# CapAI/ship-sim-gym

Hardware: AMD Instinct MI355X
Metric: env steps/sec (batched ShipEnv) (higher is better)
Workload: dtype f64

## Files before the change

### ship_sim_gym_amd/csrc/shipsim_kernels.hip

```cpp
#include <hip/hip_runtime.h>

#include <cfloat>
#include <cstdint>
#include <type_traits>

#include "shipsim.h"
#include "shipsim_internal.h"

namespace ssg {

__device__ __forceinline__ double *lds_base()
{
    extern __shared__ double s_lds[];
    return s_lds;
}

__device__ __forceinline__ double dmin(double a, double b) { return __builtin_fmin(a, b); }
__device__ __forceinline__ double dmax(double a, double b) { return __builtin_fmax(a, b); }

__device__ __forceinline__ double obs_fma(double a, double b, double c)
{
#ifndef SSG_NO_LIDAR_FMA
    return __builtin_fma(a, b, c);
#else
// ... 93 lines not shown
            const double dx = px - x, dy = py - y;
            const double d = obs_fma(dx, dx, dy * dy);
            const bool take = ((gm >> g) & 1u) & (d < best);
            best = take ? d : best;
            gi = take ? g : gi;
        }
        if (gi >= 0) { gx = hG[(2 * gi) * ld]; gy = hG[(2 * gi + 1) * ld]; }
        return;
    }
    for (int g = 0; g < c.n_goals; ++g) {
        const double px = goal_at<LDS_BANK, DYN>(c, goff, g, 0);
        const double py = goal_at<LDS_BANK, DYN>(c, goff, g, 1);
        const double dx = px - x, dy = py - y;
        const double d = obs_fma(dx, dx, dy * dy);
        const bool take = ((gm >> g) & 1u) & (d < best);
        best = take ? d : best;
        gi = take ? g : gi;
    }
    if (gi >= 0) { gx = goal_at<LDS_BANK, DYN>(c, goff, gi, 0); gy = goal_at<LDS_BANK, DYN>(c, goff, gi, 1); }
}

__device__ __forceinline__ void nearest_goal_regs(int n_goals, unsigned gm, double x, double y, const double *gp, double &gx, double &gy)
{
    gx = -1.0;
    gy = -1.0;
    double best = INFINITY;
#pragma unroll
    for (int g = 0; g < SSG_MAX_GOALS; ++g) {
        const double px = gp[2 * g], py = gp[2 * g + 1];
        const double dx = px - x, dy = py - y;
        const double d = obs_fma(dx, dx, dy * dy);
        const bool take = (g < n_goals) & (bool)((gm >> g) & 1u) & (d < best);
        best = take ? d : best;
        gx = take ? px : gx;
        gy = take ? py : gy;
    }
}

__device__ __forceinline__ int next_map(const DevCfg &c, int map_id, int env)
{
    if (c.map_ring > 0) {
        const int base = env * c.map_ring;
        const int nxt = map_id + 1;
        return (nxt - base >= c.map_ring) ? base : nxt;
    }
    const int nxt = map_id + 1;
    return (nxt >= c.n_maps) ? 0 : nxt;
}

__device__ __forceinline__ void beam_end(double cx, double cy, double ca, double sa, double cphi, double sphi, double dist,
                                         double &ex, double &ey)
{
    const double ux = obs_fma(ca, cphi, -(sa * sphi)), uy = obs_fma(sa, cphi, ca * sphi);
    ex = obs_fma(dist, ux, cx);
    ey = obs_fma(dist, uy, cy);
}

__host__ __device__ __forceinline__ constexpr int nb_lo(int nb) { return (nb + 1) / 2; }
constexpr int kBeamTabBytes = 2 * SSG_MAX_BEAMS * 8;
constexpr int kShipTabBytes = 6 * 8 * 8;
constexpr int kTrafficTabBytes = SSG_N_TRAFFIC * 4 * 8 * 8;
constexpr int kPoseDoubles = 7;
constexpr int kGoalScratchBytes = 64 * SSG_MAX_GOALS * 2 + 64 * 4;
constexpr int kTrafficScratchBytes = 64 * SSG_N_TRAFFIC * 2 + 64 * 4;
__host__ __device__ __forceinline__ constexpr int lds_fixed_bytes(int epw, bool dyn)
{
    return kBeamTabBytes + kShipTabBytes + (dyn ? kTrafficTabBytes : 0) + kPoseDoubles * epw * 8 + (dyn ? 8 : 6) * epw * 4 + 4 * (epw / 64) * 4 +
           (epw / 64) * (kGoalScratchBytes + (dyn ? kTrafficScratchBytes : 0));
}
__host__ __device__ __forceinline__ constexpr int lds_res_bytes(int nb) { return nb * 64 * 8; }
__host__ __device__ __forceinline__ constexpr int lds_queue_bytes(int nb0) { return (2 * nb0 * 64 + 64) * 2; }
__host__ __device__ __forceinline__ constexpr int lds_tile_bytes(int nb)
{
    return 2 * lds_res_bytes(nb) + 2 * lds_queue_bytes(nb_lo(nb));
}

constexpr int kHdrLidar = 10, kHdrGoals = 2 * SSG_MAX_GOALS;
static_assert(SSG_MAP_OFF_COUNTS == 0 && SSG_MAP_OFF_AABB == 2 && SSG_MAP_OFF_GOALS == kHdrLidar && SSG_MAP_OFF_SPAWN_GOAL == kHdrLidar + kHdrGoals,
              "the record's head: counts, boxes, goals, spawn goal");
#ifndef SSG_SIX_ROLE_MAX_EPW
#define SSG_SIX_ROLE_MAX_EPW 128
#endif
__host__ __device__ __forceinline__ constexpr int tile_roles(int epw, bool dyn) { return (epw <= SSG_SIX_ROLE_MAX_EPW && !dyn) ? 6 : 4; }
__host__ __device__ __forceinline__ constexpr int lds_hdr_bytes(int epw, bool lds_bank, bool dyn) { return lds_bank ? 0 : ((tile_roles(epw, dyn) - 2) * kHdrLidar + kHdrGoals) * epw * 8; }

constexpr unsigned long long kLidarMiss = ~0ull;

template <bool LDS_BANK> struct PlaneChunk { static constexpr int n = LDS_BANK ? 4 : 8; };

template <bool EXACT>
__device__ __forceinline__ double seg_mad(double a, double b, double c) { return EXACT ? a * b + c : obs_fma(a, b, c); }

template <bool LDS_BANK, bool EXACT>
__device__ __forceinline__ void lidar_pass(const DevCfg &c, const int n_items, const unsigned short *queue,
                                           unsigned long long *res , const double *beamtab,
                                           const double cx, const double cy, const double ca, const double sa,
                                           const int rec_off, const int lane, const double *hLt = nullptr , const int ld = 0)
{
    for (int base = 0; base < n_items; base += 64) {
        const int idx = base + lane;
        const bool act = idx < n_items;
        const unsigned code = queue[act ? idx : 0];
        const int src = code & 63, bi = (code >> 6) & (SSG_MAX_BEAMS - 1), s = (code >> 10) & 1;
        const double wcx = __shfl(cx, src), wcy = __shfl(cy, src), wca = __shfl(ca, src), wsa = __shfl(sa, src);
        const int woff = __shfl(rec_off, src);
        double ex, ey;
        beam_end(wcx, wcy, wca, wsa, beamtab[bi], beamtab[SSG_MAX_BEAMS + bi], c.lidar_dist, ex, ey);
        int cnt;
        if constexpr (LDS_BANK) cnt = (int)bank_at<LDS_BANK>(c, woff + SSG_MAP_OFF_COUNTS + s);
        else cnt = (int)hLt[s * ld + src];
        const int pb = woff + SSG_MAP_OFF_PLANES + s * (SSG_MAX_HULL * SSG_PLANE_DOUBLES);
        bool outside = false;
        bool out_sure = false, maybe = false;
        constexpr double kSignEps = 1e-9;
        bool ok = false;
        double ptx = ex, pty = ey;
        double bd = -1.0, bden = 1.0, t_hit = 0.0;
        int bj = 0;
        constexpr int kPlaneChunk = PlaneChunk<LDS_BANK>::n;
        for (int j0 = 0; __any(act & (j0 < cnt)); j0 += kPlaneChunk) {
            double pv0x[kPlaneChunk], pv0y[kPlaneChunk], pnx[kPlaneChunk], pny[kPlaneChunk], pv0n[kPlaneChunk];
            double pdtmin[kPlaneChunk], pdtmax[kPlaneChunk];
#pragma unroll
            for (int u = 0; u < kPlaneChunk; ++u) {
                const int j = j0 + u;
                const int q = pb + SSG_PLANE_DOUBLES * ((j < SSG_MAX_HULL) ? j : 0);
                const bool want = LDS_BANK || (act & (j < cnt));
                pv0x[u] = pv0y[u] = pnx[u] = pny[u] = pv0n[u] = 0.0;
                if (EXACT && want) { const double2 vv = bank_at2<LDS_BANK>(c, q + 0); pv0x[u] = vv.x; pv0y[u] = vv.y; }
                if (want) { const double2 nn = bank_at2<LDS_BANK>(c, q + 2); pnx[u] = nn.x; pny[u] = nn.y; }
                if (want) pv0n[u] = bank_at<LDS_BANK>(c, q + 4);
                if (EXACT) {
                    const int jp = (j == 0) ? cnt - 1 : j - 1;
                    const int qp = pb + SSG_PLANE_DOUBLES * ((jp >= 0 && jp < SSG_MAX_HULL) ? jp : 0);
                    const double ux = bank_at<LDS_BANK>(c, qp + 0), uy = bank_at<LDS_BANK>(c, qp + 1);
                    pdtmin[u] = seg_mad<EXACT>(pnx[u], uy, -(pny[u] * ux));
                    pdtmax[u] = seg_mad<EXACT>(pnx[u], pv0y[u], -(pny[u] * pv0x[u]));
                }
            }
#pragma unroll
            for (int u = 0; u < kPlaneChunk; ++u) {
                const int j = j0 + u;
                const bool valid = act & (j < cnt);
                const double nx = pnx[u], ny = pny[u], v0n = pv0n[u];
                const double an = seg_mad<EXACT>(wcx, nx, wcy * ny);
                const double d = an - v0n;
                if (EXACT) {
                    outside = outside | (valid & ((nx * (wcx - pv0x[u]) + ny * (wcy - pv0y[u])) > 0.0));
                } else {
                    out_sure = out_sure | (valid & (d > kSignEps));
                    maybe = maybe | (valid & !(d < -kSignEps));
                }
                const bool front = valid & !(d < 0.0);
                const double bn = seg_mad<EXACT>(ex, nx, ey * ny);
                const double den = dmax(an - bn, DBL_MIN);
                if (EXACT) {
                    const double t = d / den;
                    const double omt = 1.0 - t;
                    const double qx = seg_mad<EXACT>(ex, t, wcx * omt), qy = seg_mad<EXACT>(ey, t, wcy * omt);
                    const double dtv = seg_mad<EXACT>(nx, qy, -(ny * qx));
                    const bool acc = front & !((t < 0.0) | (1.0 < t)) & (pdtmin[u] <= dtv) & (dtv <= pdtmax[u]);
                    ok = ok | acc;
                    ptx = acc ? qx : ptx;
                    pty = acc ? qy : pty;
                } else {
                    const bool better = front & (d <= den) & (d * bden >= bd * den);
// ... 47 lines not shown
        }
#ifdef SSG_LIDAR_COUNT
        if (c.dbg) {
            const unsigned long long ma = __ballot(act), mh = __ballot(hit), mo = __ballot(act & !outside);
            if (lane == 0) { atomicAdd(c.dbg + 65536 + 0, (unsigned long long)__popcll(ma)); atomicAdd(c.dbg + 65536 + 1, (unsigned long long)__popcll(mh));
                             atomicAdd(c.dbg + 65536 + 2, 1ull); atomicAdd(c.dbg + 65536 + 3, (unsigned long long)__popcll(mo)); }
        }
#endif
    }
}

template <class T>
__device__ __forceinline__ void st_out(T *p, T v)
{
#ifdef SSG_WT
    __hip_atomic_store(p, v, __ATOMIC_RELAXED, __HIP_MEMORY_SCOPE_AGENT);
#else
    *p = v;
#endif
}

#ifdef SSG_STAMPS
#define SSG_STAMP(k)                                                                              \
    do {                                                                                          \
        __builtin_amdgcn_sched_barrier(0);                                                        \
        unsigned long long t_;                                                                    \
        asm volatile("s_memtime %0\n\ts_waitcnt lgkmcnt(0)" : "=s"(t_)::"memory");               \
        __builtin_amdgcn_sched_barrier(0);                                                        \
        stamp_[k] = t_;                                                                           \
    } while (0)
#define SSG_STAMP_FLUSH(n)                                                                        \
    do {                                                                                          \
        if (c.dbg && lane == 0) {                                                                 \
            unsigned long long *d_ = c.dbg + 16 * (size_t)(blockIdx.x * (NR * EPW / 64) + (threadIdx.x >> 6)); \
            for (int k_ = 0; k_ < 16; ++k_) d_[k_] = stamp_[k_];   \
        }                                                                                         \
    } while (0)
#ifdef SSG_STAMPS_ITER
#define SSG_STAMP_K(i) do { } while (0)
#else
#define SSG_STAMP_K(i) do { if (k == (K >= 2 ? K - 2 : 0)) SSG_STAMP(i); } while (0)
#endif
#else
#define SSG_STAMP(k) do { } while (0)
#define SSG_STAMP_K(i) do { } while (0)
#define SSG_STAMP_FLUSH(n) do { } while (0)
#endif

#ifdef SSG_STAMPS
#define SSG_CLOCK_BEGIN() do { } while (0)
#define SSG_CLOCK_END() do { } while (0)
#else
#define SSG_CLOCK_BEGIN() const unsigned long long clk_c0_ = __builtin_amdgcn_s_memtime(), clk_r0_ = __builtin_amdgcn_s_memrealtime()
#define SSG_CLOCK_END()                                                                            \
    do {                                                                                           \
        if (c.dbg && blockIdx.x == 0 && threadIdx.x == 0) {                                        \
            c.dbg[0] = __builtin_amdgcn_s_memtime() - clk_c0_;                                     \
            c.dbg[1] = __builtin_amdgcn_s_memrealtime() - clk_r0_;                                 \
        }                                                                                          \
    } while (0)
#endif

#ifdef SSG_ABLATION
#define SSG_ABL(bit) (c.flags & (1u << (16 + (bit))))
#else
#define SSG_ABL(bit) false
#endif

__device__ __forceinline__ void ship_world(const double *shiptab, double ca, double sa, double x, double y,
                                           double (&swx)[SSG_SHIP_VERTS], double (&swy)[SSG_SHIP_VERTS], double &sbl,
                                           double &sbr, double &sbb, double &sbt)
{
    sbl = INFINITY; sbr = -INFINITY; sbb = INFINITY; sbt = -INFINITY;
#pragma unroll
    for (int i = 0; i < SSG_SHIP_VERTS; ++i) {
        const double hx = shiptab[0 * 8 + i], hy = shiptab[1 * 8 + i];
        swx[i] = ca * hx + (-sa) * hy + x;
        swy[i] = sa * hx + ca * hy + y;
        sbl = dmin(sbl, swx[i]); sbr = dmax(sbr, swx[i]);
        sbb = dmin(sbb, swy[i]); sbt = dmax(sbt, swy[i]);
    }
}

template <int NB, bool LDS_BANK, bool EXACT>
__device__ __forceinline__ void lidar_query(const DevCfg &c, unsigned long long *res, unsigned short *queue,
                                            const double *beamtab, const int b_first, const int b_count, const double cx,
                                            const double cy, const double ca, const double sa, const int rec_off,
                                            const bool live, const int lane, const double *hL = nullptr , const int ld = 0)
{
    constexpr int NB0 = nb_lo(NB);
    constexpr int kTrash = 2 * NB0 * 64;
    int n_items = 0;
    const double eps = 1e-6;
    double al[2], ab[2], ar[2], at[2];
#pragma unroll
    for (int s = 0; s < 2; ++s) {
        double2 lb, rt;
        if constexpr (LDS_BANK) {
            lb = bank_at2<LDS_BANK>(c, rec_off + SSG_MAP_OFF_AABB + 4 * s + 0);
            rt = bank_at2<LDS_BANK>(c, rec_off + SSG_MAP_OFF_AABB + 4 * s + 2);
        } else {
            lb.x = hL[(SSG_MAP_OFF_AABB + 4 * s + 0) * ld]; lb.y = hL[(SSG_MAP_OFF_AABB + 4 * s + 1) * ld];
            rt.x = hL[(SSG_MAP_OFF_AABB + 4 * s + 2) * ld]; rt.y = hL[(SSG_MAP_OFF_AABB + 4 * s + 3) * ld];
        }
        al[s] = lb.x - eps;
        ab[s] = lb.y - eps;
        ar[s] = rt.x + eps;
        at[s] = rt.y + eps;
    }
    (void)ab; (void)at; (void)al; (void)ar;
#ifdef SSG_QUEUE_BEAM_MAJOR
#pragma unroll
    for (int k = 0; k < NB0; ++k) {
        if (k < b_count) {
            const int i = b_first + k;
            res[i * 64 + lane] = kLidarMiss;
            if (!SSG_ABL(1)) {
                double ex, ey;
                beam_end(cx, cy, ca, sa, beamtab[i], beamtab[SSG_MAX_BEAMS + i], c.lidar_dist, ex, ey);
                const double lox = dmin(cx, ex), hix = dmax(cx, ex), loy = dmin(cy, ey), hiy = dmax(cy, ey);
#pragma unroll
                for (int s = 0; s < 2; ++s) {
                    const bool need = live & (lox <= ar[s]) & (al[s] <= hix) & (loy <= at[s]) & (ab[s] <= hiy);
                    const unsigned long long m = __ballot(need);
                    const int pos = n_items + (int)__builtin_amdgcn_mbcnt_hi((unsigned)(m >> 32),
                                                                              __builtin_amdgcn_mbcnt_lo((unsigned)m, 0u));
                    queue[need ? pos : (kTrash + lane)] = (unsigned short)(lane | (k << 6) | (s << 10));
                    n_items += __popcll(m);
                }
            }
        }
    }
#else
    unsigned needmask = 0u;
    const double lca = c.lidar_dist * ca, lsa = c.lidar_dist * sa;
    const bool org0 = live & (cx <= ar[0]), org1 = live & (al[1] <= cx);
#pragma unroll
    for (int k = 0; k < NB0; ++k) {
        if (k < b_count) {
            const int i = b_first + k;
            res[i * 64 + lane] = kLidarMiss;
            if (!SSG_ABL(1)) {
                const double ex = obs_fma(lca, beamtab[i], obs_fma(-lsa, beamtab[SSG_MAX_BEAMS + i], cx));
                needmask |= (org0 | (live & (ex <= ar[0]))) ? (1u << (2 * k + 0)) : 0u;
                needmask |= (org1 | (live & (al[1] <= ex))) ? (1u << (2 * k + 1)) : 0u;
            }
        }
    }
    {
        const int cnt = __popc(needmask);
        int incl = cnt;
        incl += __builtin_amdgcn_update_dpp(0, incl, 0x111, 0xF, 0xF, false);
        incl += __builtin_amdgcn_update_dpp(0, incl, 0x112, 0xF, 0xF, false);
        incl += __builtin_amdgcn_update_dpp(0, incl, 0x114, 0xF, 0xF, false);
        incl += __builtin_amdgcn_update_dpp(0, incl, 0x118, 0xF, 0xF, false);
        incl += __builtin_amdgcn_update_dpp(0, incl, 0x142, 0xA, 0xF, false);
        incl += __builtin_amdgcn_update_dpp(0, incl, 0x143, 0xC, 0xF, false);
        n_items = __builtin_amdgcn_readlane(incl, 63);
        int pos = incl - cnt;
#pragma unroll
        for (int k = 0; k < NB0; ++k) {
            if (k < b_count) {
#pragma unroll
                for (int s = 0; s < 2; ++s) {
                    const bool need = (needmask >> (2 * k + s)) & 1u;
                    queue[need ? pos : (kTrash + lane)] = (unsigned short)(lane | (k << 6) | (s << 10));
                    pos += need ? 1 : 0;
                }
            }
        }
    }
#endif
    if (!SSG_ABL(3))
// ... 29 lines not shown

template <int NB, bool H2, int P_BEGIN, int P_END, class Val>
__device__ __forceinline__ void write_obs_tile(const ObsTile<NB> &ot, double *colbuf, const Val &val ,
                                               double *__restrict__ obase, const int rows_live, const int lane)
{
    constexpr int FF = 6 + NB;
    constexpr int DH = H2 ? 2 * FF : FF;
    constexpr int CS = ObsTile<NB>::CS, CP = ObsTile<NB>::CP;
    int lds_at[CP], gl_at[CP];
    unsigned okmask = 0;
    int ln_ = lane;
    asm volatile("" : "+v"(ln_));
#pragma unroll
    for (int jj = 0; jj < CP; ++jj) {
        lds_at[jj] = ot.lds_of(jj, ln_);
        gl_at[jj] = ot.row_of(jj, ln_) * DH + ot.col_of(jj, ln_);
        okmask |= (ot.row_of(jj, ln_) < rows_live) ? (1u << jj) : 0u;
        if constexpr (!ObsTile<NB>::kOnTheFly) asm volatile("" : "+v"(lds_at[jj]), "+v"(gl_at[jj]));
    }
    asm volatile("" : "+v"(okmask));
#pragma unroll
    for (int pi = P_BEGIN; pi < P_END; ++pi) {
        const int p0 = pi * CP;
        if (p0 >= DH) break;
        const int cpp = (DH - p0 < CP) ? (DH - p0) : CP;
#pragma unroll
        for (int cc = 0; cc < CP; ++cc) {
            if (cc < cpp) colbuf[cc * CS + lane] = val(p0 + cc);
        }
        if (cpp == CP) {
#pragma unroll
            for (int jj = 0; jj < CP; ++jj) {
                const double v = colbuf[lds_at[jj]];
                if ((okmask >> jj) & 1u) st_out(&obase[(unsigned)(gl_at[jj] + p0)], v);
            }
        } else {
            int ln = lane;
            asm volatile("" : "+v"(ln));
#pragma unroll
            for (int jj = 0; jj < CP; ++jj) {
                if (jj < cpp) {
                    const int t = ln + 64 * jj;
                    const int r = t / cpp, cc = t - r * cpp;
                    const double v = colbuf[cc * CS + r];
                    if (r < rows_live) st_out(&obase[(unsigned)(r * DH + p0 + cc)], v);
                }
            }
        }
        __builtin_amdgcn_sched_barrier(0);
    }
}

template <int NB, bool H2, int C_BEGIN, int C_END, class Val>
__device__ __forceinline__ void write_obs_pairs(double *buf , const Val &val ,
                                                double *__restrict__ obase, const int rows_live, const int lane)
{
    constexpr int FF = 6 + NB;
    constexpr int DH = H2 ? 2 * FF : FF;
    static_assert(C_BEGIN % 2 == 0 && C_END % 2 == 0 && DH % 2 == 0 && NB >= 8, "pairs of columns; 64 x 8 doubles of buffer");
    int ln = lane;
    asm volatile("" : "+v"(ln));
    const int wsw = (ln >> 2) & 3;
#pragma unroll
    for (int c0 = C_BEGIN; c0 < C_END; c0 += 8) {
        constexpr int kMax = 4;
        const int np = ((C_END - c0) / 2 < kMax) ? (C_END - c0) / 2 : kMax;
#pragma unroll
        for (int q = 0; q < kMax; ++q)
            if (q < np) *reinterpret_cast<double2 *>(buf + ln * 8 + 2 * (q ^ wsw)) = make_double2(val(c0 + 2 * q), val(c0 + 2 * q + 1));
#pragma unroll
        for (int jj = 0; jj < kMax; ++jj) {
            if (jj < np) {
                const int pidx = ln + 64 * jj;
                const int r = (np == 4) ? (pidx >> 2) : (np == 2) ? (pidx >> 1) : (np == 1) ? pidx : pidx / 3;
                const int q = pidx - r * np;
                const double2 v = *reinterpret_cast<const double2 *>(buf + r * 8 + 2 * (q ^ ((r >> 2) & 3)));
                if (r < rows_live) *reinterpret_cast<double2 *>(&obase[(unsigned)(r * DH + c0 + 2 * q)]) = v;
            }
        }
        __builtin_amdgcn_sched_barrier(0);
    }
}

template <bool LDS_BANK>
__device__ __forceinline__ bool bank_narrowphase(const DevCfg &c, const double *shiptab, const double x, const double y,
                                                 const double ca, const double sa, const int rec_off, const bool live,
                                                 const int lane, const int only ,
                                                 const double *hL = nullptr ,
                                                 const int ld = 0)
{
    const int wq = lane / 5, wi = lane - 5 * wq;
    const double w_hx = shiptab[0 * 8 + wi], w_hy = shiptab[1 * 8 + wi];
    const double w_nx = shiptab[2 * 8 + wi], w_ny = shiptab[3 * 8 + wi];
    double swx[SSG_SHIP_VERTS], swy[SSG_SHIP_VERTS], sbl, sbr, sbb, sbt;
    ship_world(shiptab, ca, sa, x, y, swx, swy, sbl, sbr, sbb, sbt);
    bool colliding = false;
    unsigned nearbits = 0;
    int cnts = 0;
#pragma unroll
    for (int s = 0; s < 2; ++s) {
        double al, ab, ar, at, cn;
        if constexpr (LDS_BANK) {
            const double2 lb = bank_at2<LDS_BANK>(c, rec_off + SSG_MAP_OFF_AABB + 4 * s + 0);
            const double2 rt = bank_at2<LDS_BANK>(c, rec_off + SSG_MAP_OFF_AABB + 4 * s + 2);
            al = lb.x; ab = lb.y; ar = rt.x; at = rt.y;
            cn = bank_at<LDS_BANK>(c, rec_off + SSG_MAP_OFF_COUNTS + s);
        } else {
            al = hL[(SSG_MAP_OFF_AABB + 4 * s + 0) * ld]; ab = hL[(SSG_MAP_OFF_AABB + 4 * s + 1) * ld];
            ar = hL[(SSG_MAP_OFF_AABB + 4 * s + 2) * ld]; at = hL[(SSG_MAP_OFF_AABB + 4 * s + 3) * ld];
            cn = hL[(SSG_MAP_OFF_COUNTS + s) * ld];
        }
        const bool near = live & !SSG_ABL(4) & ((only < 0) | (only == s)) & (sbl <= ar) & (al <= sbr);
        (void)ab; (void)at; (void)sbb; (void)sbt;
        nearbits |= near ? (1u << s) : 0u;
        cnts |= ((int)cn) << (8 * s);
    }
#pragma unroll
    for (int s = 0; s < 2; ++s) {
        const bool near_s = (nearbits >> s) & 1u;
        if (!__any(near_s)) continue;
        const int cnt = (cnts >> (8 * s)) & 0xFF;
        bool sep = false;
        if constexpr (LDS_BANK) {
            for (int j = 0; __any(near_s & !sep & (j < cnt)); ++j) {
                if (near_s & !sep & (j < cnt)) {
                    const int q = rec_off + SSG_MAP_OFF_PLANES + s * (SSG_MAX_HULL * SSG_PLANE_DOUBLES) + SSG_PLANE_DOUBLES * j;
                    const double2 nn = bank_at2<LDS_BANK>(c, q + 2);
                    const double nx = nn.x, ny = nn.y;
                    const double v0n = bank_at<LDS_BANK>(c, q + 4);
                    bool allfront = true;
#pragma unroll
                    for (int i = 0; i < SSG_SHIP_VERTS; ++i) allfront = allfront & ((nx * swx[i] + ny * swy[i]) > v0n);
                    sep = allfront;
                }
            }
        } else {
            constexpr int kNpChunk = 4;
            for (int j0 = 0; __any(near_s & !sep & (j0 < cnt)); j0 += kNpChunk) {
                if (near_s & !sep & (j0 < cnt)) {
                    double nx[kNpChunk], ny[kNpChunk], v0n[kNpChunk];
#pragma unroll
                    for (int u = 0; u < kNpChunk; ++u) {
                        const int j = (j0 + u < SSG_MAX_HULL) ? j0 + u : 0;
                        const int q = rec_off + SSG_MAP_OFF_PLANES + s * (SSG_MAX_HULL * SSG_PLANE_DOUBLES) + SSG_PLANE_DOUBLES * j;
                        const double2 nn = bank_at2<LDS_BANK>(c, q + 2);
                        nx[u] = nn.x; ny[u] = nn.y;
                        v0n[u] = bank_at<LDS_BANK>(c, q + 4);
                    }
#pragma unroll
                    for (int u = 0; u < kNpChunk; ++u) {
                        bool allfront = j0 + u < cnt;
#pragma unroll
                        for (int i = 0; i < SSG_SHIP_VERTS; ++i) allfront = allfront & ((nx[u] * swx[i] + ny[u] * swy[i]) > v0n[u]);
                        sep = sep | allfront;
                    }
                }
            }
        }
        nearbits = sep ? (nearbits & ~(1u << s)) : nearbits;
    }
    unsigned long long todo = __ballot(nearbits != 0u);
    while (todo) {
        const int src = __ffsll((long long)todo) - 1;
        todo &= todo - 1;
        const double bx = readlane_f64(x, src), by = readlane_f64(y, src);
        const double bca = readlane_f64(ca, src), bsa = readlane_f64(sa, src);
        const int boff = __builtin_amdgcn_readlane(rec_off, src);
        const unsigned bnear = (unsigned)__builtin_amdgcn_readlane((int)nearbits, src);
        const int bcnts = __builtin_amdgcn_readlane(cnts, src);
        const double svx = bca * w_hx + (-bsa) * w_hy + bx, svy = bsa * w_hx + bca * w_hy + by;
        const double snx_ = bca * w_nx + (-bsa) * w_ny, sny_ = bsa * w_nx + bca * w_ny;
        const double off_i = snx_ * svx + sny_ * svy;
        bool col = false;
#pragma unroll
        for (int s = 0; s < 2; ++s) {
            if (!(bnear & (1u << s))) continue;
            const int cnt = (bcnts >> (8 * s)) & 0xFF;
            const bool valid = (lane < 60) & (wq < cnt);
            const int q = boff + SSG_MAP_OFF_PLANES + s * (SSG_MAX_HULL * SSG_PLANE_DOUBLES) +
                          SSG_PLANE_DOUBLES * ((wq < SSG_MAX_HULL) ? wq : 0);
            const double v0x = bank_at<LDS_BANK>(c, q + 0), v0y = bank_at<LDS_BANK>(c, q + 1);
            const double nx = bank_at<LDS_BANK>(c, q + 2), ny = bank_at<LDS_BANK>(c, q + 3);
            const double v0n = bank_at<LDS_BANK>(c, q + 4);
            const bool frontA = (nx * svx + ny * svy) > v0n;
            const bool frontB = (snx_ * v0x + sny_ * v0y) > off_i;
            const unsigned long long mV = __ballot(valid);
            const unsigned long long mA = __ballot(valid & frontA);
            const unsigned long long missB = mV & ~__ballot(valid & frontB);
            const unsigned long long P = 0x0084210842108421ull;
            const unsigned long long allA = mA & (mA >> 1) & (mA >> 2) & (mA >> 3) & (mA >> 4) & P;
            bool sepB = false;
#pragma unroll
            for (int i = 0; i < SSG_SHIP_VERTS; ++i) sepB = sepB | (((missB >> i) & P) == 0ull);
            const bool separated = (allA != 0ull) | sepB;
            col = col | !separated;
        }
        colliding = (lane == src) ? col : colliding;
    }
    return colliding;
}

template <int NB, int EPW, bool LDS_BANK, bool EXACT, bool DYN>
__global__ __launch_bounds__(tile_roles(EPW, DYN) * EPW) void step_kernel(const DevCfg c, const int32_t *__restrict__ actions_kn,
                                                       double *__restrict__ obs, double *__restrict__ reward_out,
                                                       uint8_t *__restrict__ done_out, uint8_t *__restrict__ flags_out,
                                                       const int K_launch, const long long traj)
{
    const int K = DYN ? 1 : K_launch;
    SSG_CLOCK_BEGIN();
    constexpr int NB0 = nb_lo(NB);
    constexpr int NR = tile_roles(EPW, DYN);
    const int role = threadIdx.x / EPW;
    const int tl = threadIdx.x - role * EPW;
    const int e = blockIdx.x * EPW + tl;
    const bool live = e < c.n_envs;
    const int el_ = live ? e : 0;
    const size_t np = (size_t)c.n_pad;
    const int lane = threadIdx.x & 63;

    double *__restrict__ colX = c.f64cols + COL_X * np;
    double *__restrict__ colY = c.f64cols + COL_Y * np;
    double *__restrict__ colVX = c.f64cols + COL_VX * np;
    double *__restrict__ colVY = c.f64cols + COL_VY * np;
    double *__restrict__ colA = c.f64cols + COL_A * np;
    double *__restrict__ colW = c.f64cols + COL_W * np;
    double *__restrict__ colCum = c.f64cols + COL_CUM * np;
    double *__restrict__ colLid = c.f64cols + COL_LIDAR * np;
    int32_t *__restrict__ colRud = c.i32cols + ICOL_RUDDER * np;
    int32_t *__restrict__ colStep = c.i32cols + ICOL_STEP * np;
    int32_t *__restrict__ colMap = c.i32cols + ICOL_MAP * np;

    const int bank_bytes = LDS_BANK ? ((c.n_maps * (SSG_MAP_STRIDE * 8) + 15) & ~15) : 0;
    char *lds_fixed = reinterpret_cast<char *>(lds_base()) + bank_bytes;
    double *beamtab = reinterpret_cast<double *>(lds_fixed);
    double *shiptab = reinterpret_cast<double *>(lds_fixed + kBeamTabBytes);
    double *traffictab = reinterpret_cast<double *>(lds_fixed + kBeamTabBytes + kShipTabBytes);
    double *pose = reinterpret_cast<double *>(lds_fixed + kBeamTabBytes + kShipTabBytes + (DYN ? kTrafficTabBytes : 0));
    int *posem = reinterpret_cast<int *>(pose + kPoseDoubles * EPW);
    int *poser = posem + EPW;
    unsigned *gres = reinterpret_cast<unsigned *>(poser + EPW);
    unsigned *gdone = gres + 2 * EPW;
    unsigned *gtraf = gdone + 2 * EPW;
    unsigned *sync_ready = gtraf + (DYN ? 2 * EPW : 0);
    unsigned *sync_ack = sync_ready + EPW / 64;
    unsigned *sync_bar = sync_ack + EPW / 64;
    char *goal_scratch0 = reinterpret_cast<char *>(sync_bar + 2 * (EPW / 64));
    char *traffic_scratch0 = goal_scratch0 + (EPW / 64) * kGoalScratchBytes;
    char *scratch0 = lds_fixed + lds_fixed_bytes(EPW, DYN);
    char *tile_base = scratch0 + (tl >> 6) * lds_tile_bytes(NB);
    double *hdr0 = reinterpret_cast<double *>(scratch0 + (EPW / 64) * lds_tile_bytes(NB));
    double *hL = LDS_BANK ? nullptr : hdr0 + ((role & 1) + (role >= 4 ? 2 : 0)) * (kHdrLidar * EPW) + tl;
    double *hG = LDS_BANK ? nullptr : hdr0 + (NR - 2) * kHdrLidar * EPW + tl;
    auto load_hdr_lidar = [&](int rec_off) {
#pragma unroll
        for (int f = 0; f < kHdrLidar / 2; ++f) { const double2 v = bank_at2<LDS_BANK>(c, rec_off + 2 * f); hL[(2 * f) * EPW] = v.x; hL[(2 * f + 1) * EPW] = v.y; }
    };
    auto load_hdr_goals = [&](int rec_off) {
#pragma unroll
        for (int f = 0; f < kHdrGoals / 2; ++f) { const double2 v = bank_at2<LDS_BANK>(c, rec_off + SSG_MAP_OFF_GOALS + 2 * f); hG[(2 * f) * EPW] = v.x; hG[(2 * f + 1) * EPW] = v.y; }
    };

#ifdef SSG_STAMPS
    unsigned long long stamp_[16] = {};
#endif
    SSG_STAMP(8);

    double bank_tail_v = 0.0;
    int bank_tail_o = -1;
    if (LDS_BANK && !SSG_ABL(8)) stage_bank_lds<NR * EPW>(c.bank, c.n_maps * (SSG_MAP_STRIDE * 8), bank_tail_v, bank_tail_o);
    double tv[6] = {0.0, 0.0, 0.0, 0.0, 0.0, 0.0};
    if (threadIdx.x < 2 * SSG_MAX_BEAMS)
        tv[0] = (threadIdx.x < SSG_MAX_BEAMS) ? c.beam_cos[threadIdx.x & (SSG_MAX_BEAMS - 1)] : c.beam_sin[threadIdx.x & (SSG_MAX_BEAMS - 1)];
    if (threadIdx.x >= 64 && threadIdx.x < 64 + SSG_SHIP_VERTS) {
        const int i = threadIdx.x - 64, ip = (i == 0) ? (SSG_SHIP_VERTS - 1) : (i - 1);
        tv[0] = c.hull[2 * i]; tv[1] = c.hull[2 * i + 1]; tv[2] = c.nrm[2 * i]; tv[3] = c.nrm[2 * i + 1]; tv[4] = c.hull[2 * ip]; tv[5] = c.hull[2 * ip + 1];
    }
    if constexpr (DYN) {
        if (threadIdx.x >= 160 && threadIdx.x < 160 + SSG_N_TRAFFIC * SSG_SHIP_VERTS) {
            const int kk = (threadIdx.x - 160) / SSG_SHIP_VERTS, i = (threadIdx.x - 160) % SSG_SHIP_VERTS;
            tv[0] = c.thull[kk][2 * i]; tv[1] = c.thull[kk][2 * i + 1]; tv[2] = c.tnrm[kk][2 * i]; tv[3] = c.tnrm[kk][2 * i + 1];
        }
    }
    auto flush_tables = [&]() {
        if (bank_tail_o >= 0) *reinterpret_cast<double *>(reinterpret_cast<char *>(lds_base()) + bank_tail_o) = bank_tail_v;
        if (threadIdx.x < 2 * SSG_MAX_BEAMS) beamtab[threadIdx.x] = tv[0];
        if (threadIdx.x >= 64 && threadIdx.x < 64 + SSG_SHIP_VERTS) {
            const int i = threadIdx.x - 64;
            shiptab[0 * 8 + i] = tv[0]; shiptab[1 * 8 + i] = tv[1];
            shiptab[2 * 8 + i] = tv[2]; shiptab[3 * 8 + i] = tv[3];
            shiptab[4 * 8 + i] = tv[4]; shiptab[5 * 8 + i] = tv[5];
        }
        if constexpr (DYN) {
            if (threadIdx.x >= 160 && threadIdx.x < 160 + SSG_N_TRAFFIC * SSG_SHIP_VERTS) {
                const int kk = (threadIdx.x - 160) / SSG_SHIP_VERTS, i = (threadIdx.x - 160) % SSG_SHIP_VERTS;
                traffictab[(kk * 4 + 0) * 8 + i] = tv[0]; traffictab[(kk * 4 + 1) * 8 + i] = tv[1];
                traffictab[(kk * 4 + 2) * 8 + i] = tv[2]; traffictab[(kk * 4 + 3) * 8 + i] = tv[3];
            }
        }
    };
    if (threadIdx.x == 128) {
        double bl = INFINITY, br = -INFINITY, bb = INFINITY, bt = -INFINITY;
        for (int i = 0; i < SSG_SHIP_VERTS; ++i) {
            const double hx = c.hull[2 * i], hy = c.hull[2 * i + 1];
            const double wx = 1.0 * hx + (-0.0) * hy + c.spawn_x, wy = 0.0 * hx + 1.0 * hy + c.spawn_y;
            bl = dmin(bl, wx); br = dmax(br, wx); bb = dmin(bb, wy); bt = dmax(bt, wy);
        }
        shiptab[0 * 8 + 6] = c.spawn_x + (br - bl) / 2;
        shiptab[1 * 8 + 6] = c.spawn_y + (bt - bb) / 2;
    }
    if (threadIdx.x >= 192 && threadIdx.x < 192 + 4 * (EPW / 64)) sync_ready[threadIdx.x - 192] = 0u;
    const bool auto_reset = (c.flags & SSG_FLAG_AUTO_RESET) != 0u;
    const int tile = tl >> 6;
    auto wait_pose = [&](int k) {
        while (__hip_atomic_load(&sync_ready[tile], __ATOMIC_ACQUIRE, __HIP_MEMORY_SCOPE_WORKGROUP) != (unsigned)(k + 1))
            __builtin_amdgcn_s_sleep(2);
    };
    auto ack_pose = [&]() {
        if (lane == 0) __hip_atomic_fetch_add(&sync_ack[tile], 1u, __ATOMIC_RELEASE, __HIP_MEMORY_SCOPE_WORKGROUP);
    };
    unsigned *sync_q = sync_bar + EPW / 64;
    auto query_done = [&]() {
        if (lane == 0) __hip_atomic_fetch_add(&sync_q[tile], 1u, __ATOMIC_RELEASE, __HIP_MEMORY_SCOPE_WORKGROUP);
    };
    auto wait_queries = [&]() {
        while (__hip_atomic_load(&sync_q[tile], __ATOMIC_ACQUIRE, __HIP_MEMORY_SCOPE_WORKGROUP) < 2u)
            __builtin_amdgcn_s_sleep(1);
    };
    auto tile_barrier = [&](int k) {
        if (lane == 0) __hip_atomic_fetch_add(&sync_bar[tile], 1u, __ATOMIC_RELEASE, __HIP_MEMORY_SCOPE_WORKGROUP);
        while (__hip_atomic_load(&sync_bar[tile], __ATOMIC_ACQUIRE, __HIP_MEMORY_SCOPE_WORKGROUP) < (unsigned)NR * (unsigned)(k + 1))
            __builtin_amdgcn_s_sleep(1);
    };

    auto traffic_collide = [&](auto k0_, auto k1_, const double *tpre, double x, double y, double ca, double sa, int part,
                               unsigned short *tq , unsigned *tw ) {
        constexpr int K0 = decltype(k0_)::value, K1 = decltype(k1_)::value;
        const int wq = lane / 5, wi = lane - 5 * wq;
        const double w_hx = shiptab[0 * 8 + wi], w_hy = shiptab[1 * 8 + wi], w_nx = shiptab[2 * 8 + wi], w_ny = shiptab[3 * 8 + wi];
        double sbl, sbr, sbb, sbt;
        {
            double swx[SSG_SHIP_VERTS], swy[SSG_SHIP_VERTS];
            ship_world(shiptab, ca, sa, x, y, swx, swy, sbl, sbr, sbb, sbt);
        }
        tw[lane] = 0u;
        int n_tp = 0;
#pragma unroll
        for (int kk = K0; kk < K1; ++kk) {
            const double tx = tpre[4 * kk + 0], ty = tpre[4 * kk + 1];
            const double dx = dmax(dmax(sbl - tx, tx - sbr), 0.0), dy = dmax(dmax(sbb - ty, ty - sbt), 0.0);
            bool cand = false;
            if (live & ((dx * dx + dy * dy) <= c.dyn_reach2[kk])) {
                const double tca = tpre[4 * kk + 2], tsa = tpre[4 * kk + 3];
                double bl = INFINITY, br = -INFINITY, bb = INFINITY, bt = -INFINITY;
#pragma unroll
                for (int i = 0; i < SSG_SHIP_VERTS; ++i) {
                    const double gx = traffictab[(kk * 4 + 0) * 8 + i], gy = traffictab[(kk * 4 + 1) * 8 + i];
                    const double wx = tca * gx + (-tsa) * gy + tx, wy = tsa * gx + tca * gy + ty;
                    bl = dmin(bl, wx); br = dmax(br, wx); bb = dmin(bb, wy); bt = dmax(bt, wy);
                }
                cand = (sbl <= br) & (bl <= sbr) & (sbb <= bt) & (bb <= sbt);
            }
            const unsigned long long m = __ballot(cand);
            const int pos = n_tp + (int)__builtin_amdgcn_mbcnt_hi((unsigned)(m >> 32), __builtin_amdgcn_mbcnt_lo((unsigned)m, 0u));
            if (cand) tq[pos] = (unsigned short)(lane | (kk << 6));
            n_tp += __popcll(m);
        }
        for (int base = 0; base < n_tp; base += 12) {
            const int p = base + wq;
            const bool valid = (lane < 60) & (p < n_tp);
            const unsigned code = tq[valid ? p : 0];
            const int src = code & 63, kk = code >> 6;
            const double bx = __shfl(x, src), by = __shfl(y, src), bca = __shfl(ca, src), bsa = __shfl(sa, src);
            double tx = __shfl(tpre[4 * K0 + 0], src), ty = __shfl(tpre[4 * K0 + 1], src), tca = __shfl(tpre[4 * K0 + 2], src), tsa = __shfl(tpre[4 * K0 + 3], src);
#pragma unroll
            for (int h = K0 + 1; h < K1; ++h) {
                const double a0 = __shfl(tpre[4 * h + 0], src), a1 = __shfl(tpre[4 * h + 1], src);
                const double a2 = __shfl(tpre[4 * h + 2], src), a3 = __shfl(tpre[4 * h + 3], src);
                tx = (kk == h) ? a0 : tx; ty = (kk == h) ? a1 : ty; tca = (kk == h) ? a2 : tca; tsa = (kk == h) ? a3 : tsa;
            }
            const double *tt = traffictab + kk * 32;
            bool sep;
            {
                const double nx = bca * w_nx + (-bsa) * w_ny, ny = bsa * w_nx + bca * w_ny;
                const double vx_ = bca * w_hx + (-bsa) * w_hy + bx, vy_ = bsa * w_hx + bca * w_hy + by;
                const double off = nx * vx_ + ny * vy_;
                double mn = INFINITY;
#pragma unroll
                for (int j = 0; j < SSG_SHIP_VERTS; ++j) {
                    const double gx = tt[0 * 8 + j], gy = tt[1 * 8 + j];
                    const double qx = tca * gx + (-tsa) * gy + tx, qy = tsa * gx + tca * gy + ty;
                    mn = dmin(mn, nx * qx + ny * qy);
                }
                sep = mn > off;
            }
            {
                const double lnx = tt[2 * 8 + wi], lny = tt[3 * 8 + wi], lvx = tt[0 * 8 + wi], lvy = tt[1 * 8 + wi];
                const double nx = tca * lnx + (-tsa) * lny, ny = tsa * lnx + tca * lny;
                const double vx_ = tca * lvx + (-tsa) * lvy + tx, vy_ = tsa * lvx + tca * lvy + ty;
                const double off = nx * vx_ + ny * vy_;
                double mn = INFINITY;
#pragma unroll
                for (int j = 0; j < SSG_SHIP_VERTS; ++j) {
                    const double hx = shiptab[0 * 8 + j], hy = shiptab[1 * 8 + j];
                    const double qx = bca * hx + (-bsa) * hy + bx, qy = bsa * hx + bca * hy + by;
                    mn = dmin(mn, nx * qx + ny * qy);
                }
                sep |= mn > off;
            }
            const unsigned long long ms = __ballot(valid & sep);
            const bool separated = ((ms >> (5 * wq)) & 31ull) != 0ull;
            if (valid & (wi == 0) & !separated) atomicOr(&tw[src], 1u);
        }
        gtraf[part * EPW + tl] = (tw[lane] != 0u) ? 1u : 0u;
    };
    auto traffic_hit = [&](int) -> unsigned { return gtraf[tl] | gtraf[EPW + tl]; };
    if (role < 2) {
        unsigned short *queue = reinterpret_cast<unsigned short *>(tile_base + 2 * lds_res_bytes(NB) + role * lds_queue_bytes(NB0));
        const int b_first = role ? NB0 : 0, b_count = role ? (NB - NB0) : NB0;
        double ca, sa, cx, cy;
        int map_id;
        double tpre[DYN ? 4 * SSG_N_TRAFFIC : 1] = {};
        {
            const double x = colX[el_], y = colY[el_], ang = colA[el_];
            map_id = colMap[el_];
            if constexpr (!LDS_BANK) load_hdr_lidar(map_id * SSG_MAP_STRIDE);
            { const double2 sc = sincos_call(ang); sa = sc.x; ca = sc.y; }
            if (role == 0) { pose[2 * EPW + tl] = ca; pose[3 * EPW + tl] = sa; }
            flush_tables();
            if (LDS_BANK) __builtin_amdgcn_s_waitcnt(0);
            __syncthreads();
            SSG_STAMP(9);
            if constexpr (DYN) {
                {
                    const double *tcol = c.dyn_f64 + (size_t)DC_TRAFFIC * np, *trot = c.dyn_f64 + (size_t)DC_TROT * np;
#pragma unroll
                    for (int kk = 0; kk < SSG_N_TRAFFIC; ++kk) {
                        if ((kk == 0) != (role == 0)) continue;
                        tpre[4 * kk + 0] = tcol[(size_t)(9 * kk) * np + el_]; tpre[4 * kk + 1] = tcol[(size_t)(9 * kk + 1) * np + el_];
                        tpre[4 * kk + 2] = trot[(size_t)(2 * kk) * np + el_]; tpre[4 * kk + 3] = trot[(size_t)(2 * kk + 1) * np + el_];
                    }
                }
            }
            double swx[SSG_SHIP_VERTS], swy[SSG_SHIP_VERTS], bl, br, bb, bt;
            ship_world(shiptab, ca, sa, x, y, swx, swy, bl, br, bb, bt);
            cx = x + (br - bl) / 2;
            cy = y + (bt - bb) / 2;
        }
        lidar_query<NB, LDS_BANK, EXACT>(c, reinterpret_cast<unsigned long long *>(tile_base), queue, beamtab, b_first, b_count,
                                         cx, cy, ca, sa, map_id * SSG_MAP_STRIDE, live, lane, hL, EPW);
        if (K == 1) query_done();
        for (int k = 0; k < K; ++k) {
            if constexpr (NR == 4) wait_pose(k);
            if constexpr (DYN) {
#pragma unroll
                for (int i = 0; i < 4 * SSG_N_TRAFFIC; ++i) asm volatile("" : "+v"(tpre[i]));
            }
            SSG_STAMP_K(0);
            double nca = 0.0, nsa = 0.0, ncx = 0.0, ncy = 0.0, npx = 0.0, npy = 0.0;
            int nmap = 0;
            if constexpr (NR == 4) {
                nca = pose[2 * EPW + tl]; nsa = pose[3 * EPW + tl];
                ncx = pose[4 * EPW + tl]; ncy = pose[5 * EPW + tl];
                npx = pose[0 * EPW + tl]; npy = pose[1 * EPW + tl];
                nmap = posem[tl];
                ack_pose();
                reinterpret_cast<unsigned short *>(gres)[2 * ((k & 1) * EPW + tl) + role] =
                        bank_narrowphase<LDS_BANK>(c, shiptab, npx, npy, nca, nsa, nmap * SSG_MAP_STRIDE, live, lane, role, hL, EPW) ? 1 : 0;
            }
            SSG_STAMP_K(4);
            if constexpr (DYN) {
                static_assert(lds_queue_bytes(1) >= 64 * 2 + 64 * 4, "lidar-lo's pair queue holds ship 0's pair queue and hit words");
                unsigned short *tq1 = reinterpret_cast<unsigned short *>(traffic_scratch0 + (tl >> 6) * kTrafficScratchBytes);
                if (role == 0) traffic_collide(std::integral_constant<int, 0>{}, std::integral_constant<int, 1>{}, tpre, npx, npy, nca, nsa, 0,
                                               queue, reinterpret_cast<unsigned *>(queue + 64));
                else traffic_collide(std::integral_constant<int, 1>{}, std::integral_constant<int, SSG_N_TRAFFIC>{}, tpre, npx, npy, nca, nsa, 1,
                                     tq1, reinterpret_cast<unsigned *>(tq1 + 64 * SSG_N_TRAFFIC));
            }

            SSG_STAMP_K(3);
            tile_barrier(k);
            SSG_STAMP_K(1);
            if constexpr (NR == 6) {
                if (k + 1 < K) {
                    nca = pose[2 * EPW + tl]; nsa = pose[3 * EPW + tl];
                    ncx = pose[4 * EPW + tl]; ncy = pose[5 * EPW + tl];
                    nmap = posem[tl];
                    ack_pose();
                }
            }
            if (k + 1 < K) {
                const bool rs = auto_reset & ((gres[(k & 1) * EPW + tl] | (gdone[(k & 1) * EPW + tl] & 1u) | (DYN ? traffic_hit(k) : 0u)) != 0u);
                ca = rs ? 1.0 : nca; sa = rs ? 0.0 : nsa;
                cx = rs ? shiptab[0 * 8 + 6] : ncx; cy = rs ? shiptab[1 * 8 + 6] : ncy;
                map_id = rs ? next_map(c, nmap, el_) : nmap;
                if constexpr (!LDS_BANK) {
                    if (rs) load_hdr_lidar(map_id * SSG_MAP_STRIDE);
                }
                lidar_query<NB, LDS_BANK, EXACT>(c, reinterpret_cast<unsigned long long *>(tile_base + ((k + 1) & 1) * lds_res_bytes(NB)),
                                                 queue, beamtab, b_first, b_count, cx, cy, ca, sa, map_id * SSG_MAP_STRIDE, live, lane, hL, EPW);
                if (k + 1 == K - 1) query_done();
            }
            SSG_STAMP_K(2);
        }
        if (K == 1 && live) {
            const bool rs = auto_reset & ((gres[tl] | (gdone[tl] & 1u) | (DYN ? traffic_hit(0) : 0u)) != 0u);
            const unsigned long long *rk = reinterpret_cast<const unsigned long long *>(tile_base);
            for (int kb = 0; kb < b_count; ++kb) {
                const int i = b_first + kb;
                const unsigned long long key = rk[i * 64 + lane];
                const double hitd = __longlong_as_double((long long)(key & 0x7FFFFFFFFFFFFFFFull));
                if (rs | (key != kLidarMiss)) st_out(&colLid[(size_t)i * np + el_], rs ? -1.0 : hitd);
            }
        }
        SSG_STAMP(10);
        SSG_STAMP_FLUSH(3);
        SSG_CLOCK_END();
        return;
    }

    if constexpr (NR == 6) {
        if (role >= 4) {
            const int h = role - 4;
            int map0 = colMap[el_];
            if constexpr (!LDS_BANK) load_hdr_lidar(map0 * SSG_MAP_STRIDE);
            asm volatile("" : "+v"(map0));
            flush_tables();
            if (LDS_BANK) __builtin_amdgcn_s_waitcnt(0);
            __syncthreads();
            SSG_STAMP(9);
            for (int k = 0; k < K; ++k) {
                wait_pose(k);
                SSG_STAMP_K(0);
                const double nca = pose[2 * EPW + tl], nsa = pose[3 * EPW + tl];
                const double npx = pose[0 * EPW + tl], npy = pose[1 * EPW + tl];
                const int nmap = posem[tl];
                ack_pose();
                reinterpret_cast<unsigned short *>(gres)[2 * ((k & 1) * EPW + tl) + h] =
                        bank_narrowphase<LDS_BANK>(c, shiptab, npx, npy, nca, nsa, nmap * SSG_MAP_STRIDE, live, lane, h, hL, EPW) ? 1 : 0;
                SSG_STAMP_K(1);
                tile_barrier(k);
                SSG_STAMP_K(2);
                if constexpr (!LDS_BANK) {
                    if (k + 1 < K) {
                        const bool rs = auto_reset & ((gres[(k & 1) * EPW + tl] | (gdone[(k & 1) * EPW + tl] & 1u)) != 0u);
                        if (rs) load_hdr_lidar(next_map(c, nmap, el_) * SSG_MAP_STRIDE);
                    }
                }
            }
            SSG_STAMP(10);
            SSG_STAMP_FLUSH(5);
            return;
        }
    }

    const int wq = lane / 5, wi = lane - 5 * wq;

    if (role == 2) {
        constexpr int F = 6 + NB;
        double pv[F];
        double ogp[DYN ? 2 * SSG_MAX_GOALS : 1];
        unsigned gm_pre = 0u;
        {
            const int el = el_;
            const double x0 = colX[el], y0 = colY[el], a0 = colA[el];
            const int rud0 = colRud[el], map0 = colMap[el];
            const unsigned gm0 = c.mask[el];
#pragma unroll
            for (int i = 0; i < NB; ++i) pv[6 + i] = colLid[(size_t)i * np + el];
            pv[0] = x0; pv[1] = y0; pv[2] = (double)rud0; pv[3] = a0;
            if constexpr (DYN) {
                pv[4] = c.dyn_f64[(size_t)(DC_PREV_GOAL + 0) * np + el];
                pv[5] = c.dyn_f64[(size_t)(DC_PREV_GOAL + 1) * np + el];
            }
#pragma unroll
            for (int i = 0; i < 4; ++i) asm volatile("" : "+v"(pv[i]));
#pragma unroll
            for (int i = 0; i < NB; ++i) asm volatile("" : "+v"(pv[6 + i]));
            if constexpr (DYN) asm volatile("" : "+v"(pv[4]), "+v"(pv[5]));
            int map0_ = map0; unsigned gm0_ = gm0;
            asm volatile("" : "+v"(map0_), "+v"(gm0_));
            gm_pre = gm0_;
// ... 780 lines not shown
```

Before: 13.45 billion.

## Give lidar to one wave and fuse both hulls' collision into another wave

```diff
diff --git a/ship_sim_gym_amd/csrc/shipsim_kernels.hip b/ship_sim_gym_amd/csrc/shipsim_kernels.hip
--- a/ship_sim_gym_amd/csrc/shipsim_kernels.hip
+++ b/ship_sim_gym_amd/csrc/shipsim_kernels.hip
@@ -199,6 +199,12 @@
 #define SSG_SIX_ROLE_MAX_EPW 128
 #endif
 __host__ __device__ __forceinline__ constexpr int tile_roles(int epw, bool dyn) { return (epw <= SSG_SIX_ROLE_MAX_EPW && !dyn) ? 6 : 4; }
+#ifdef SSG_LIDAR_SPLIT_BEAMS
+constexpr bool kLidarSplitBeams = true;
+#else
+constexpr bool kLidarSplitBeams = false;
+#endif
+__host__ __device__ __forceinline__ constexpr bool lidar_one_wave(int epw, bool dyn) { return !kLidarSplitBeams && !dyn && tile_roles(epw, dyn) == 4; }
 __host__ __device__ __forceinline__ constexpr int lds_hdr_bytes(int epw, bool lds_bank, bool dyn) { return lds_bank ? 0 : ((tile_roles(epw, dyn) - 2) * kHdrLidar + kHdrGoals) * epw * 8; }
 
 constexpr unsigned long long kLidarMiss = ~0ull;
@@ -412,13 +418,14 @@
     }
 }
 
-template <int NB, bool LDS_BANK, bool EXACT>
+template <int NBQ, bool LDS_BANK, bool EXACT>
 __device__ __forceinline__ void lidar_query(const DevCfg &c, unsigned long long *res, unsigned short *queue,
                                             const double *beamtab, const int b_first, const int b_count, const double cx,
                                             const double cy, const double ca, const double sa, const int rec_off,
                                             const bool live, const int lane, const double *hL = nullptr , const int ld = 0)
 {
-    constexpr int NB0 = nb_lo(NB);
+    static_assert(NBQ >= 1 && NBQ <= SSG_MAX_BEAMS && SSG_MAX_BEAMS == 16, "a beam index in four bits of the item code, 2 x NBQ <= 32 bits of needmask");
+    constexpr int NB0 = NBQ;
     constexpr int kTrash = 2 * NB0 * 64;
     int n_items = 0;
     const double eps = 1e-6;
@@ -614,7 +621,12 @@
     }
 }
 
-template <bool LDS_BANK>
+#ifdef SSG_COLLIDE_PER_HULL
+constexpr bool kCollideFused = false;
+#else
+constexpr bool kCollideFused = true;
+#endif
+template <bool LDS_BANK, bool FUSED = false>
 __device__ __forceinline__ bool bank_narrowphase(const DevCfg &c, const double *shiptab, const double x, const double y,
                                                  const double ca, const double sa, const int rec_off, const bool live,
                                                  const int lane, const int only ,
@@ -647,6 +659,45 @@
         nearbits |= near ? (1u << s) : 0u;
         cnts |= ((int)cn) << (8 * s);
     }
+    if constexpr (FUSED) {
+#ifdef SSG_COLLIDE_NP
+        constexpr int kNp = SSG_COLLIDE_NP;
+#else
+        constexpr int kNp = LDS_BANK ? 2 : 4;
+#endif
+        unsigned left = nearbits;
+#ifdef SSG_COLLIDE_DIRECT_MAX
+        if (__popcll(__ballot(nearbits != 0u)) <= SSG_COLLIDE_DIRECT_MAX) left = 0u;
+#endif
+        for (int round = 0; round < 2 && __any(left != 0u); ++round) {
+            const bool mine = left != 0u;
+            const int s = (left & 1u) ? 0 : 1;
+            const int cnt = (cnts >> (8 * s)) & 0xFF;
+            const int pb = rec_off + SSG_MAP_OFF_PLANES + s * (SSG_MAX_HULL * SSG_PLANE_DOUBLES);
+            bool sep = false;
+            for (int j0 = 0; __any(mine & !sep & (j0 < cnt)); j0 += kNp) {
+                if (mine & !sep & (j0 < cnt)) {
+                    double nx[kNp], ny[kNp], v0n[kNp];
+#pragma unroll
+                    for (int u = 0; u < kNp; ++u) {
+                        const int q = pb + SSG_PLANE_DOUBLES * ((j0 + u < SSG_MAX_HULL) ? j0 + u : 0);
+                        const double2 nn = bank_at2<LDS_BANK>(c, q + 2);
+                        nx[u] = nn.x; ny[u] = nn.y;
+                        v0n[u] = bank_at<LDS_BANK>(c, q + 4);
+                    }
+#pragma unroll
+                    for (int u = 0; u < kNp; ++u) {
+                        bool allfront = j0 + u < cnt;
+#pragma unroll
+                        for (int i = 0; i < SSG_SHIP_VERTS; ++i) allfront = allfront & ((nx[u] * swx[i] + ny[u] * swy[i]) > v0n[u]);
+                        sep = sep | allfront;
+                    }
+                }
+            }
+            nearbits = (mine & sep) ? (nearbits & ~(1u << s)) : nearbits;
+            left &= ~(1u << s);
+        }
+    } else {
 #pragma unroll
     for (int s = 0; s < 2; ++s) {
         const bool near_s = (nearbits >> s) & 1u;
@@ -690,6 +741,7 @@
             }
         }
         nearbits = sep ? (nearbits & ~(1u << s)) : nearbits;
+    }
     }
     unsigned long long todo = __ballot(nearbits != 0u);
     while (todo) {
@@ -850,12 +902,13 @@
     auto ack_pose = [&]() {
         if (lane == 0) __hip_atomic_fetch_add(&sync_ack[tile], 1u, __ATOMIC_RELEASE, __HIP_MEMORY_SCOPE_WORKGROUP);
     };
+    constexpr bool kOneLidar = lidar_one_wave(EPW, DYN);
     unsigned *sync_q = sync_bar + EPW / 64;
     auto query_done = [&]() {
         if (lane == 0) __hip_atomic_fetch_add(&sync_q[tile], 1u, __ATOMIC_RELEASE, __HIP_MEMORY_SCOPE_WORKGROUP);
     };
     auto wait_queries = [&]() {
-        while (__hip_atomic_load(&sync_q[tile], __ATOMIC_ACQUIRE, __HIP_MEMORY_SCOPE_WORKGROUP) < 2u)
+        while (__hip_atomic_load(&sync_q[tile], __ATOMIC_ACQUIRE, __HIP_MEMORY_SCOPE_WORKGROUP) < (kOneLidar ? 1u : 2u))
             __builtin_amdgcn_s_sleep(1);
     };
     auto tile_barrier = [&](int k) {
@@ -946,9 +999,46 @@
         gtraf[part * EPW + tl] = (tw[lane] != 0u) ? 1u : 0u;
     };
     auto traffic_hit = [&](int) -> unsigned { return gtraf[tl] | gtraf[EPW + tl]; };
+    if constexpr (kOneLidar) {
+        if (role == 1) {
+            int map0 = colMap[el_];
+            if constexpr (!LDS_BANK) load_hdr_lidar(map0 * SSG_MAP_STRIDE);
+            asm volatile("" : "+v"(map0));
+            flush_tables();
+            if (LDS_BANK) __builtin_amdgcn_s_waitcnt(0);
+            __syncthreads();
+            SSG_STAMP(9);
+            for (int k = 0; k < K; ++k) {
+                wait_pose(k);
+                SSG_STAMP_K(0);
+                const double nca = pose[2 * EPW + tl], nsa = pose[3 * EPW + tl];
+                const double npx = pose[0 * EPW + tl], npy = pose[1 * EPW + tl];
+                const int nmap = posem[tl];
+                ack_pose();
+                gres[(k & 1) * EPW + tl] =
+                        bank_narrowphase<LDS_BANK, kCollideFused>(c, shiptab, npx, npy, nca, nsa, nmap * SSG_MAP_STRIDE, live, lane, -1, hL, EPW) ? 1u : 0u;
+                SSG_STAMP_K(4);
+                SSG_STAMP_K(3);
+                tile_barrier(k);
+                SSG_STAMP_K(1);
+                if constexpr (!LDS_BANK) {
+                    if (k + 1 < K) {
+                        const bool rs = auto_reset & ((gres[(k & 1) * EPW + tl] | (gdone[(k & 1) * EPW + tl] & 1u)) != 0u);
+                        if (rs) load_hdr_lidar(next_map(c, nmap, el_) * SSG_MAP_STRIDE);
+                    }
+                }
+                SSG_STAMP_K(2);
+            }
+            SSG_STAMP(10);
+            SSG_STAMP_FLUSH(3);
+            return;
+        }
+    }
     if (role < 2) {
-        unsigned short *queue = reinterpret_cast<unsigned short *>(tile_base + 2 * lds_res_bytes(NB) + role * lds_queue_bytes(NB0));
-        const int b_first = role ? NB0 : 0, b_count = role ? (NB - NB0) : NB0;
+        constexpr int NBQ = kOneLidar ? NB : NB0;
+        static_assert(2 * lds_queue_bytes(NB0) >= (2 * NB * 64 + 64) * 2, "the tile's two pair queues hold one queue of all beams x both hulls + trash");
+        unsigned short *queue = reinterpret_cast<unsigned short *>(tile_base + 2 * lds_res_bytes(NB) + (kOneLidar ? 0 : role) * lds_queue_bytes(NB0));
+        const int b_first = (!kOneLidar && role) ? NB0 : 0, b_count = kOneLidar ? NB : (role ? (NB - NB0) : NB0);
         double ca, sa, cx, cy;
         int map_id;
         double tpre[DYN ? 4 * SSG_N_TRAFFIC : 1] = {};
@@ -978,7 +1068,7 @@
             cx = x + (br - bl) / 2;
             cy = y + (bt - bb) / 2;
         }
-        lidar_query<NB, LDS_BANK, EXACT>(c, reinterpret_cast<unsigned long long *>(tile_base), queue, beamtab, b_first, b_count,
+        lidar_query<NBQ, LDS_BANK, EXACT>(c, reinterpret_cast<unsigned long long *>(tile_base), queue, beamtab, b_first, b_count,
                                          cx, cy, ca, sa, map_id * SSG_MAP_STRIDE, live, lane, hL, EPW);
         if (K == 1) query_done();
         for (int k = 0; k < K; ++k) {
@@ -996,8 +1086,10 @@
                 npx = pose[0 * EPW + tl]; npy = pose[1 * EPW + tl];
                 nmap = posem[tl];
                 ack_pose();
-                reinterpret_cast<unsigned short *>(gres)[2 * ((k & 1) * EPW + tl) + role] =
-                        bank_narrowphase<LDS_BANK>(c, shiptab, npx, npy, nca, nsa, nmap * SSG_MAP_STRIDE, live, lane, role, hL, EPW) ? 1 : 0;
+                if constexpr (!kOneLidar)
+                    reinterpret_cast<unsigned short *>(gres)[2 * ((k & 1) * EPW + tl) + role] =
+                            bank_narrowphase<LDS_BANK>(c, shiptab, npx, npy, nca, nsa, nmap * SSG_MAP_STRIDE, live, lane, role, hL, EPW) ? 1 : 0;
+                (void)npx; (void)npy;
             }
             SSG_STAMP_K(4);
             if constexpr (DYN) {
@@ -1028,7 +1120,7 @@
                 if constexpr (!LDS_BANK) {
                     if (rs) load_hdr_lidar(map_id * SSG_MAP_STRIDE);
                 }
-                lidar_query<NB, LDS_BANK, EXACT>(c, reinterpret_cast<unsigned long long *>(tile_base + ((k + 1) & 1) * lds_res_bytes(NB)),
+                lidar_query<NBQ, LDS_BANK, EXACT>(c, reinterpret_cast<unsigned long long *>(tile_base + ((k + 1) & 1) * lds_res_bytes(NB)),
                                                  queue, beamtab, b_first, b_count, cx, cy, ca, sa, map_id * SSG_MAP_STRIDE, live, lane, hL, EPW);
                 if (k + 1 == K - 1) query_done();
             }
```

After: 13.65 billion (median of 6 runs). +1.5%, better.
